# m-schuetz/SimLOD

Measured on NVIDIA H100. Metric: Mpoints/sec octree insertion (16B XYZRGBA), higher is better.
Workload: dtype u32+f32

## Files before the change

### simlod_b200/csrc/construct.cu

```cuda
#include <cooperative_groups.h>
#include <stdint.h>
#include "../../include/simlod_abi.h"
#include "fpmath.cuh"

namespace cg = cooperative_groups;

typedef SimlodPoint Point;
typedef SimlodChunk Chunk;
typedef SimlodNode Node;
typedef SimlodStats Stats;
typedef SimlodUniforms Uniforms;
typedef SimlodHeapHeader Heap;
struct CudaPrint;

#include "construct_layout.cuh"

enum : uint32_t {
    ERR_SPILL_OVERFLOW  = 1u << 0,
    ERR_VOXEL_OVERFLOW  = 1u << 1,
    ERR_DIR_OVERFLOW    = 1u << 2,
    ERR_NODE_OVERFLOW   = 1u << 3,
    ERR_QUEUE_OVERFLOW  = 1u << 4,
    ERR_SPILLNODE_OVERFLOW = 1u << 5,
    ERR_ROW_OVERFLOW    = 1u << 6,
// ... 254 lines not shown
}

constexpr uint32_t PROVISIONAL = 0x80000000u;
static_assert(scratch::ITEM_CAP < (1u << 24), "block-local ranks must fit 24 bits");
constexpr uint32_t CHILD_RANK_BITS = 11;
constexpr uint32_t CHILD_SLOTS = 64 * 8;
__shared__ uint32_t sh_childCount[CHILD_SLOTS];
__shared__ uint8_t  sh_childSplit[CHILD_SLOTS];
__shared__ uint32_t sh_roundSplits;
__device__ __forceinline__ uint32_t childWord(uint32_t e, uint32_t rank) { return PROVISIONAL | (e << CHILD_RANK_BITS) | rank; }
__device__ __forceinline__ uint32_t childOf(uint32_t sl) { return (sl >> CHILD_RANK_BITS) & (CHILD_SLOTS - 1u); }
__device__ __forceinline__ uint32_t finalChildSlot(uint32_t sl) { return (sl & PROVISIONAL) ? sh_childCount[childOf(sl)] + (sl & ((1u << CHILD_RANK_BITS) - 1u)) : sl; }
__shared__ uint32_t sh_leafKey[VOXTAB_SIZE];
__shared__ uint32_t sh_leafCount[VOXTAB_SIZE];
__shared__ uint32_t sh_leafBase[VOXTAB_SIZE];
__shared__ uint8_t  sh_leafLevel[VOXTAB_SIZE];
__device__ __forceinline__ uint32_t finalSlot(uint32_t sl) { return (sl & PROVISIONAL) ? sh_leafBase[(sl >> 24) & 127u] + (sl & 0xffffffu) : sl; }
constexpr uint32_t RUNSLOT_CAP = 2048;
__shared__ uint32_t sh_runSlot[RUNSLOT_CAP];
constexpr uint32_t LIST_CAP = 2048;
static_assert(LIST_CAP <= (1u << CHILD_RANK_BITS), "a child's block-local ranks must fit its slot word");
__shared__ uint32_t sh_listCount;
__shared__ uint32_t sh_listMode;
__shared__ uint32_t sh_blockLegacy;
__shared__ uint8_t  sh_entrySplit[VOXTAB_SIZE];
constexpr uint32_t WL_SPLIT_SHIFT = 22;
constexpr uint32_t WL_ITEM_MASK = (1u << WL_SPLIT_SHIFT) - 1u;
static_assert(scratch::ITEM_CAP <= (1u << WL_SPLIT_SHIFT), "worklist entries keep the item in 22 bits");
__shared__ uint32_t sh_splitNodes[64];
__shared__ SpillInfo sh_splitInfo[64];
__shared__ uint32_t sh_splitGranule[65];
__shared__ uint32_t sh_wlCount, sh_wlBase, sh_wlFill;
__shared__ uint32_t sh_roundLegacy, sh_roundListed;
__device__ __forceinline__ uint32_t blockExclusiveScan(uint32_t v, uint32_t& total) {
    __shared__ uint32_t sh_warpSum[8];
    __shared__ uint32_t sh_total;
    const uint32_t lane = laneId(), warp = threadIdx.x >> 5;
    uint32_t incl = v;
#pragma unroll
    for (int o = 1; o < 32; o <<= 1) { uint32_t t = __shfl_up_sync(0xffffffffu, incl, o); if (lane >= (uint32_t)o) incl += t; }
    __syncthreads();
    if (lane == 31) sh_warpSum[warp] = incl;
    __syncthreads();
    if (threadIdx.x == 0) { uint32_t run = 0; for (int w = 0; w < 8; w++) { uint32_t t = sh_warpSum[w]; sh_warpSum[w] = run; run += t; } sh_total = run; }
    __syncthreads();
    total = sh_total;
    return sh_warpSum[warp] + incl - v;
}

constexpr uint32_t BLOOM_WORDS = 8;
constexpr uint32_t AFFECTED_CAP = 1024;
__shared__ uint32_t sh_runBloom[BLOOM_WORDS];
__shared__ uint32_t sh_affected[AFFECTED_CAP];
__shared__ uint32_t sh_numAffected;
__device__ __forceinline__ uint32_t bloomHash(uint32_t node) { return (node * 0x9E3779B1u) >> 24; }
__device__ __forceinline__ void bloomAdd(uint32_t* bloom, uint32_t node) { uint32_t h = bloomHash(node); atomicOr(&bloom[h >> 5], 1u << (h & 31u)); }

struct Rewalk { uint32_t perRun, runItems, total, spilledBefore; bool listed; };
__device__ __forceinline__ Rewalk rewalkSlice(uint32_t numBatch, uint32_t numSpilled, uint32_t spilledBefore) {
    Rewalk r;
    r.perRun = ((numBatch + gridDim.x - 1) / gridDim.x + 31u) & ~31u;
    r.listed = gridDim.x <= AFFECTED_CAP;
    r.runItems = (r.listed ? sh_numAffected : gridDim.x) * r.perRun;
    r.total = r.runItems + numSpilled;
    r.spilledBefore = spilledBefore;
    return r;
// ... 237 lines not shown
        asm volatile("{\n\t.reg .pred p;\n\tmbarrier.try_wait.parity.shared::cta.b64 p, [%1], %2;\n\tselp.u32 %0, 1, 0, p;\n\t}"
                     : "=r"(done) : "r"(bar), "r"(parity) : "memory");
    } while (!done);
}

__device__ __forceinline__ void blockRun(uint32_t numBatch, uint32_t& first, uint32_t& end) {
    const uint32_t perBlock = ((numBatch + gridDim.x - 1) / gridDim.x + 31u) & ~31u;
    first = min(numBatch, blockIdx.x * perBlock);
    end = min(numBatch, first + perBlock);
}

__device__ __forceinline__ void markAffectedRun(const Ctx& c, const Batch& b, uint32_t spillBegin, uint32_t spillEnd) {
    if (threadIdx.x >= 32) return;
    const uint32_t perRun = ((b.size + gridDim.x - 1) / gridDim.x + 31u) & ~31u;
    uint32_t flag = 0;
    if (blockIdx.x * perRun < b.size) {
        const uint32_t* bloom = c.runBloom() + blockIdx.x * BLOOM_WORDS;
        for (uint32_t k = spillBegin + threadIdx.x; k < spillEnd; k += 32) {
            const uint32_t h = bloomHash(c.spill()[k].node);
            flag |= (ldcg(&bloom[h >> 5]) >> (h & 31u)) & 1u;
        }
        flag = __any_sync(0xffffffffu, flag != 0) ? 1u : 0u;
    }
    if (threadIdx.x == 0) c.runFlag()[blockIdx.x] = flag;
}

__device__ __forceinline__ uint32_t* listItem() { return reinterpret_cast<uint32_t*>(&sh_tile[0][0]); }
__device__ __forceinline__ uint32_t* listSlot() { return reinterpret_cast<uint32_t*>(&sh_tile[0][0]) + LIST_CAP; }
static_assert(sizeof(sh_tile) >= LIST_CAP * 8, "the explicit item list must fit the TMA stages");

__device__ void buildWorklist(const Ctx& c, const Batch& b, uint32_t spillBegin, uint32_t spillEnd, uint32_t round) {
    Ctl::Worklist* w = &c.ctl()->wl[b.index % 3u];
    const uint32_t numSplit = spillEnd - spillBegin;
#ifdef SIMLOD_NO_WORKLIST
    if (true) {
#else
    if (numSplit > 64u || sh_blockLegacy != 0) {
#endif
        if (threadIdx.x == 0) atomicExch(&w->legacy, 1u);
        return;
    }
    uint32_t blockFirst, blockEnd;
    blockRun(b.size, blockFirst, blockEnd);
    const uint32_t mode = sh_listMode;
    const uint32_t total = mode == 0 ? blockEnd - blockFirst : min(sh_listCount, LIST_CAP);
    if (threadIdx.x == 0) { sh_wlCount = 0; sh_wlFill = 0; }
    if (mode == 0) {
        if (threadIdx.x < numSplit) sh_splitNodes[threadIdx.x] = c.spill()[spillBegin + threadIdx.x].node;
        __syncthreads();
        if (threadIdx.x < VOXTAB_SIZE) {
            const uint32_t key = sh_leafKey[threadIdx.x];
            uint32_t f = 0;
            if (key != VOXTAB_EMPTY) for (uint32_t j = 0; j < numSplit; j++) f = key == sh_splitNodes[j] ? j + 1u : f;
            sh_entrySplit[threadIdx.x] = (uint8_t)f;
        }
    } else {
        for (uint32_t e = threadIdx.x; e < CHILD_SLOTS; e += blockDim.x) sh_childSplit[e] = 0;
        __syncthreads();
        if (threadIdx.x < numSplit) {
            const uint32_t node = c.spill()[spillBegin + threadIdx.x].node;
            for (uint32_t k = 0; k < sh_roundSplits; k++) {
                const uint32_t o = node - sh_splitInfo[k].childBase;
                if (o < 8u) sh_childSplit[k * 8u + o] = (uint8_t)(threadIdx.x + 1u);
            }
        }
    }
    __syncthreads();
    const uint32_t* words = mode == 0 ? sh_runSlot : listSlot();
    auto splitOf = [&](uint32_t word) -> uint32_t {
        if ((word & PROVISIONAL) == 0) return 0u;
        return mode == 0 ? sh_entrySplit[(word >> 24) & (VOXTAB_SIZE - 1)] : sh_childSplit[childOf(word)];
    };
    auto movedAt = [&](uint32_t k) { return splitOf(words[k]) != 0; };
    auto wlSplit = [&](uint32_t word) { return (splitOf(word) - 1u) << WL_SPLIT_SHIFT; };
    uint32_t cnt = 0;
    for (uint32_t k = threadIdx.x; k < total; k += blockDim.x) cnt += movedAt(k) ? 1u : 0u;
    for (int o = 16; o > 0; o >>= 1) cnt += __shfl_xor_sync(0xffffffffu, cnt, o);
    if (laneId() == 0 && cnt) atomicAdd(&sh_wlCount, cnt);
    __syncthreads();
    if (threadIdx.x == 0) {
        const uint32_t n = sh_wlCount;
        uint32_t base = n ? atomicAdd(&w->cursor[round & 1u], n) : 0u;
        if ((uint64_t)base + n > scratch::WL_CAP) { atomicExch(&w->legacy, 1u); base = 0xffffffffu; }
        sh_wlBase = base;
    }
    __syncthreads();
    const uint32_t base = sh_wlBase;
    if (base == 0xffffffffu || sh_wlCount == 0) return;
    uint32_t* wl = c.worklist();
    const uint32_t* items = listItem();
    for (uint32_t k0 = 0; k0 < total; k0 += blockDim.x) {
        const uint32_t k = k0 + threadIdx.x;
        const bool m = k < total && movedAt(k);
        const uint32_t mask = __ballot_sync(0xffffffffu, m);
        if (mask == 0) continue;
        uint32_t off = 0;
        if (laneId() == 0) off = atomicAdd(&sh_wlFill, (uint32_t)__popc(mask));
        off = __shfl_sync(0xffffffffu, off, 0);
        if (m) wl[base + off + __popc(mask & lanemaskLt())] = (mode == 0 ? blockFirst + k : items[k]) | wlSplit(words[k]);
    }
}

template <bool SAMPLE, bool COUNT, bool FRESH, bool UNCACHED_GRID>
__device__ __forceinline__ void passItems(const Ctx& c, const Batch& b, uint32_t numSpilled, uint32_t spilledBefore, uint32_t round, uint32_t spillBegin = 0, uint32_t spillEnd = 0) {
    uint32_t blockFirst, blockEnd;
    blockRun(b.size, blockFirst, blockEnd);
    LeafCache cache;
    cache.leaf = VOXTAB_EMPTY; cache.parent = VOXTAB_EMPTY; cache.key = 0;

    if (COUNT && threadIdx.x < VOXTAB_SIZE) { sh_leafKey[threadIdx.x] = VOXTAB_EMPTY; sh_leafCount[threadIdx.x] = 0; }
    if (FRESH && COUNT && threadIdx.x < BLOOM_WORDS) sh_runBloom[threadIdx.x] = 0;
    if (FRESH && COUNT && threadIdx.x == 0) { sh_listMode = 0; sh_listCount = 0; sh_blockLegacy = (blockEnd - blockFirst) > RUNSLOT_CAP ? 1u : 0u; }
    if (SAMPLE) voxelPassBegin(c, b, FRESH);
    __syncthreads();

    if (FRESH) {
        const uint32_t runLen = blockEnd - blockFirst;
        const uint32_t numTiles = (runLen + TILE_POINTS - 1) / TILE_POINTS;
        __syncthreads();
        if (threadIdx.x == 0) asm volatile("fence.proxy.async.shared::cta;" ::: "memory");
        if (threadIdx.x == 0 && numTiles > 0) tileLoad(0, b.points + blockFirst, min(TILE_POINTS, runLen));
        for (uint32_t t = 0; t < numTiles; t++) {
            const uint32_t tileFirst = blockFirst + t * TILE_POINTS;
            if (threadIdx.x == 0 && t + 1 < numTiles)
                tileLoad((t + 1) & 1, b.points + tileFirst + TILE_POINTS, min(TILE_POINTS, blockEnd - (tileFirst + TILE_POINTS)));
            tileWait(t & 1, sh_tilePhase[t & 1] ^ ((t >> 1) & 1u));
#pragma unroll 1
            for (uint32_t k = 0; k < TILE_POINTS / 256; k++) {
                const uint32_t idx = k * 256 + threadIdx.x;
                const uint32_t i = tileFirst + idx;
                const bool valid = i < blockEnd;
                uint4 pt = valid ? sh_tile[t & 1][idx] : make_uint4(0, 0, 0, 0);
                uint32_t lp = 0, slot = 0;
                walk<SAMPLE, COUNT, UNCACHED_GRID, true>(c, b, cache, valid, pt, 0, 0, 0, COUNT ? sh_runBloom : nullptr, false, lp, slot);
                if (valid && COUNT) {
                    c.leafOf(b.parity)[i] = lp;
                    if (runLen <= RUNSLOT_CAP) sh_runSlot[i - blockFirst] = slot; else c.slotOf(b.parity)[i] = slot;
                }
            }
            __syncthreads();
        }
        if (threadIdx.x == 0) { sh_tilePhase[0] ^= ((numTiles + 1) >> 1) & 1u; sh_tilePhase[1] ^= (numTiles >> 1) & 1u; }
        if (COUNT && threadIdx.x < BLOOM_WORDS) c.runBloom()[blockIdx.x * BLOOM_WORDS + threadIdx.x] = sh_runBloom[threadIdx.x];
    } else {
        uint32_t* leafOf = c.leafOf(b.parity);
        uint32_t* slotOf = c.slotOf(b.parity);
        if (sh_roundLegacy == 0) {
            const uint32_t listed = min(sh_roundListed, (uint32_t)scratch::WL_CAP);
            const uint32_t perRun = ((b.size + gridDim.x - 1) / gridDim.x + 31u) & ~31u;
            const uint32_t numSplit = spillEnd - spillBegin;
            if (threadIdx.x < numSplit) sh_splitInfo[threadIdx.x] = c.spill()[spillBegin + threadIdx.x];
            for (uint32_t e = threadIdx.x; e < CHILD_SLOTS; e += blockDim.x) sh_childCount[e] = 0;
            if (threadIdx.x == 0) { sh_listCount = 0; sh_listMode = 1; sh_roundSplits = numSplit; }
            __syncthreads();
            if (threadIdx.x == 0) {
                uint32_t run = 0;
                for (uint32_t k = 0; k < numSplit; k++) { sh_splitGranule[k] = run; run += (sh_splitInfo[k].stored + 31u) / 32u; }
                sh_splitGranule[numSplit] = run;
            }
            __syncthreads();
#if SIMLOD_TIMERS >= 2
            uint64_t tRw = globaltimer();
#define RW_DONE(k) do { __syncthreads(); if (blockIdx.x == 0 && threadIdx.x == 0) { uint64_t _t = globaltimer(); c.ctl()->subNanos[k] += _t - tRw; tRw = _t; } } while (0)
#else
#define RW_DONE(k) do { } while (0)
#endif
            auto reserve = [&](bool valid, bool& forceGlobal) {
                const uint32_t vmask = __ballot_sync(0xffffffffu, valid);
                uint32_t k0 = 0;
                if (laneId() == 0) k0 = atomicAdd(&sh_listCount, (uint32_t)__popc(vmask));
                k0 = __shfl_sync(0xffffffffu, k0, 0);
                forceGlobal = k0 + __popc(vmask) > LIST_CAP;
                if (forceGlobal && laneId() == 0) atomicAdd(&c.ctl()->events[1], 1u);
                return k0 + __popc(vmask & lanemaskLt());
            };
            auto remember = [&](uint32_t i, uint32_t lp, uint32_t slot, uint32_t myk, bool forceGlobal) {
                leafOf[i] = lp;
                if (!forceGlobal) { listItem()[myk] = i; listSlot()[myk] = slot; }
                else {
                    slotOf[i] = slot;
                    if (myk < LIST_CAP) { listItem()[myk] = 0xffffffffu; listSlot()[myk] = 0; }
                }
            };
            RW_DONE(12);
            constexpr uint32_t NO_ITEM = 0xffffffffu;
            auto sampleSplitLeaf = [&](uint64_t grid, const Coords& q, uint32_t color, uint32_t node, uint32_t level) {
                if (!nested(q)) atomicOr(&c.ctl()->errorFlags, ERR_FAR_POINT);
                const uint32_t cell = cellAt(q, level);
                uint32_t* word = reinterpret_cast<uint32_t*>(grid) + (cell >> 5);
                const uint32_t bit = 1u << (cell & 31u);
                const uint32_t seen = (UNCACHED_GRID || SIMLOD_REWALK_L2TEST) ? ldcg(word) : *word;
                if ((seen & bit) == 0 && (atomicOr(word, bit) & bit) == 0) recordVoxel(c, b, node, cell, color);
            };
            {
                const uint32_t share = ((listed + gridDim.x - 1) / gridDim.x + 31u) & ~31u;
                const uint32_t first = min(listed, blockIdx.x * share);
                const uint32_t numListed = min(listed - first, share);
                const uint32_t* wl = c.worklist() + first;
                const uint32_t stride = blockDim.x;
                auto loadEntry = [&](uint32_t bs) { const uint32_t u = bs + laneId(); return u < numListed ? wl[u] : NO_ITEM; };
                auto loadPoint = [&](uint32_t e) {
                    const uint32_t i = e & WL_ITEM_MASK;
                    if (e == NO_ITEM) return make_uint4(0, 0, 0, 0);
                    return i >= scratch::MAX_BATCH ? *reinterpret_cast<const uint4*>(c.spilled() + (i - scratch::MAX_BATCH)) : ldPoint(b.points + i);
                };
                uint32_t base = threadIdx.x & ~31u;
                uint32_t eCur = loadEntry(base), eNext = loadEntry(base + stride);
                uint4 ptCur = loadPoint(eCur);
                for (; base < numListed; base += stride) {
                    const uint4 ptNext = loadPoint(eNext);
                    const uint32_t eNext2 = loadEntry(base + 2u * stride);
                    const uint32_t i = eCur & WL_ITEM_MASK, k = eCur >> WL_SPLIT_SHIFT;
                    const uint4 pt = ptCur;
                    bool valid = eCur != NO_ITEM;
                    const bool spilledItem = valid && i >= scratch::MAX_BATCH;
                    uint32_t node = 0, level = 0, childBase = 0;
                    uint64_t grid = 0;
                    if (valid) {
                        if (k < numSplit) { node = sh_splitInfo[k].node; level = sh_splitInfo[k].level; childBase = sh_splitInfo[k].childBase; grid = sh_splitInfo[k].grid; }
                        else { valid = false; atomicOr(&c.ctl()->errorFlags, ERR_INTERNAL); }
                        valid = valid && level < SIMLOD_MAX_DEPTH;
                    }
                    if (__any_sync(0xffffffffu, valid)) {
                        bool forceGlobal;
                        const uint32_t myk = reserve(valid, forceGlobal);
                        const Coords q = quantize(c, pt);
                        const uint32_t octant = childIndexAt(q, level);
                        const uint32_t child = childBase + octant;
                        if (SAMPLE && valid) sampleSplitLeaf(grid, q, pt.w, node, level);
                        __syncwarp();
                        uint32_t slot = 0;
                        if (COUNT) {
                            uint32_t* bloom = valid && !spilledItem ? c.runBloom() + (i / perRun) * BLOOM_WORDS : nullptr;
                            slot = countChild<false, true>(valid, k * 8u + octant, child, level + 1, bloom, forceGlobal);
                        }
                        if (valid && COUNT) remember(i, child | ((level + 1) << 24), slot, myk, forceGlobal);
                    }
                    eCur = eNext; ptCur = ptNext; eNext = eNext2;
                }
            }
            RW_DONE(13);
            {
                const uint32_t allGranules = sh_splitGranule[numSplit];
                const uint32_t share = (allGranules + gridDim.x - 1) / gridDim.x;
                const uint32_t gFirst = min(allGranules, blockIdx.x * share);
                const uint32_t numGranules = min(allGranules - gFirst, share);
                const uint32_t gStride = blockDim.x / 32u;
                struct Granule { uint32_t lo, j; bool valid; };
                auto locate = [&](uint32_t g) {
                    Granule r; r.lo = 0; r.j = 0; r.valid = false;
                    if (g < numGranules) {
                        const uint32_t ga = gFirst + g;
                        uint32_t lo = 0, hi = numSplit;
                        while (hi - lo > 1) { const uint32_t mid = (lo + hi) >> 1; if (sh_splitGranule[mid] <= ga) lo = mid; else hi = mid; }
                        const uint32_t within = (ga - sh_splitGranule[lo]) * 32u + laneId();
                        r.lo = lo; r.j = sh_splitInfo[lo].base + within;
                        r.valid = within < sh_splitInfo[lo].stored && sh_splitInfo[lo].level < SIMLOD_MAX_DEPTH;
                    }
                    return r;
                };
                auto loadSpilled = [&](const Granule& gr) { return gr.valid ? *reinterpret_cast<const uint4*>(c.spilled() + gr.j) : make_uint4(0, 0, 0, 0); };
                uint32_t g = threadIdx.x >> 5;
                Granule cur = locate(g);
                uint4 ptCur = loadSpilled(cur);
                for (; g < numGranules; g += gStride) {
                    const Granule next = locate(g + gStride);
                    const uint4 ptNext = loadSpilled(next);
                    const bool valid = cur.valid;
                    if (__any_sync(0xffffffffu, valid)) {
                        const uint32_t node = sh_splitInfo[cur.lo].node, level = sh_splitInfo[cur.lo].level, childBase = sh_splitInfo[cur.lo].childBase;
                        const uint32_t i = (uint32_t)scratch::MAX_BATCH + cur.j;
                        const uint4 pt = ptCur;
                        bool forceGlobal;
                        const uint32_t myk = reserve(valid, forceGlobal);
                        const Coords q = quantize(c, pt);
                        const uint32_t octant = childIndexAt(q, level);
                        const uint32_t child = childBase + octant;
                        if (SAMPLE && valid) sampleSplitLeaf(sh_splitInfo[cur.lo].grid, q, pt.w, node, level);
                        __syncwarp();
                        uint32_t slot = 0;
                        if (COUNT) slot = countChild<true, false>(valid, cur.lo * 8u + octant, child, level + 1, nullptr, forceGlobal);
                        if (valid && COUNT) remember(i, child | ((level + 1) << 24), slot, myk, forceGlobal);
                    }
                    cur = next; ptCur = ptNext;
                }
            }
            RW_DONE(14);
        } else {
            if (threadIdx.x == 0) sh_blockLegacy = 1;
            if (first_in_grid()) atomicAdd(&c.ctl()->events[0], 1u);
            if (gridDim.x <= AFFECTED_CAP) {
                const uint32_t* flags = c.runFlag();
                uint32_t numAffected = 0;
                for (uint32_t g0 = 0; g0 < gridDim.x; g0 += blockDim.x) {
                    const uint32_t g = g0 + threadIdx.x;
                    const uint32_t flag = g < gridDim.x ? ldcg(&flags[g]) : 0u;
                    uint32_t total = 0;
                    const uint32_t off = blockExclusiveScan(flag, total);
                    if (flag) sh_affected[numAffected + off] = g;
                    numAffected += total;
                }
                if (threadIdx.x == 0) sh_numAffected = numAffected;
                __syncthreads();
            }
            const Rewalk rw = rewalkSlice(b.size, numSpilled, spilledBefore);
            for (uint32_t base = rewalkFirstGranule(); base < rw.total; base += rewalkGranuleStride()) {
                const uint32_t u = base + laneId();
                uint32_t run = 0xffffffffu, i = 0xffffffffu, node = 0, level = 0;
                bool valid = u < rw.total;
                const bool spilledItem = valid && u >= rw.runItems;
                if (valid) { i = rewalkItem(rw, u, run); valid = spilledItem || i < b.size; }
                uint4 pt = make_uint4(0, 0, 0, 0);
                if (spilledItem) pt = *reinterpret_cast<const uint4*>(c.spilled() + (i - scratch::MAX_BATCH));
                if (valid) {
                    uint32_t lp = leafOf[i];
                    node = lp & 0xffffffu; level = lp >> 24;
                    if (!(spilledItem && i - scratch::MAX_BATCH >= rw.spilledBefore)) valid = c.firstChild()[node] != 0 && level < SIMLOD_MAX_DEPTH;
                }
                if (!__any_sync(0xffffffffu, valid)) continue;
                if (valid && !spilledItem) pt = ldPoint(b.points + i);
// ... 60 lines not shown
                if (sl & PROVISIONAL) slotOf[i] = finalSlot(sl);
            }
        }
    }
    __syncthreads();
}

constexpr uint32_t SPLIT_COPY_PARTS = 256, SPLIT_CLEAR_PARTS = 32, SPLIT_PARTS = SPLIT_COPY_PARTS + SPLIT_CLEAR_PARTS + 1;

__device__ __noinline__ void splitRound(uint32_t begin, uint32_t end) {
    const Ctx c;
    const Batch& b = sh_batch;
    const uint32_t numWarps = (gridDim.x * blockDim.x) >> 5;
    const uint32_t warp = (threadIdx.x >> 5) * gridDim.x + blockIdx.x;
    const uint32_t lane = laneId();
    const uint32_t numItems = (end - begin) * SPLIT_PARTS;
    uint32_t* leafOf = c.leafOf(b.parity);
    for (uint32_t item = warp; item < numItems; item += numWarps) {
        const SpillInfo info = c.spill()[begin + item / SPLIT_PARTS];
        const uint32_t part = item % SPLIT_PARTS;
        const uint32_t numChunks = (info.stored + SIMLOD_POINTS_PER_CHUNK - 1) / SIMLOD_POINTS_PER_CHUNK;
        if (part < SPLIT_COPY_PARTS) {
            const uint32_t k = part >> 2, quarter = part & 3u;
            if (k >= numChunks || info.row == 0) continue;
            const Chunk* chunk = reinterpret_cast<const Chunk*>(c.rows()[(uint64_t)(info.row - 1) * scratch::ROW_SLOTS + k]);
            const uint32_t inChunk = min((uint32_t)SIMLOD_POINTS_PER_CHUNK, info.stored - k * SIMLOD_POINTS_PER_CHUNK);
            const uint32_t first = quarter * 256u;
            const uint32_t n = inChunk > first ? min(256u, inChunk - first) : 0u;
            const uint32_t tag = info.node | (info.level << 24);
            const uint4* src = reinterpret_cast<const uint4*>(&chunk->points[first]);
            const uint32_t dst = info.base + k * SIMLOD_POINTS_PER_CHUNK + first;
#pragma unroll 1
            for (uint32_t h = 0; h < 256u; h += 128u) {
                uint4 v[4];
#pragma unroll
                for (int u = 0; u < 4; u++) if (h + lane + 32u * u < n) v[u] = src[h + lane + 32u * u];
#pragma unroll
                for (int u = 0; u < 4; u++) if (h + lane + 32u * u < n) {
                    *reinterpret_cast<uint4*>(c.spilled() + dst + h + lane + 32u * u) = v[u];
                    leafOf[scratch::MAX_BATCH + dst + h + lane + 32u * u] = tag;
                }
            }
        } else if (part < SPLIT_COPY_PARTS + SPLIT_CLEAR_PARTS) {
            constexpr uint32_t PER = SIMLOD_GRID_WORDS / 4 / SPLIT_CLEAR_PARTS;
            uint4* g = reinterpret_cast<uint4*>(info.grid) + (uint64_t)(part - SPLIT_COPY_PARTS) * PER;
#pragma unroll 4
            for (uint32_t i = lane; i < PER; i += 32) g[i] = make_uint4(0, 0, 0, 0);
        } else {
            Node* parent = &c.nodes()[info.node];
            const uint32_t pX = parent->X, pY = parent->Y, pZ = parent->Z;
            if (lane < 8) {
                Node* child = &c.nodes()[info.childBase + lane];
                uint64_t* raw = reinterpret_cast<uint64_t*>(child);
#pragma unroll
                for (int w = 0; w < 19; w++) raw[w] = 0;
                child->level = info.level + 1;
                child->X = 2 * pX + ((lane >> 2) & 1);
                child->Y = 2 * pY + ((lane >> 1) & 1);
                child->Z = 2 * pZ + (lane & 1);
                for (int k = 0; k < 20; k++) child->name[k] = parent->name[k];
                reinterpret_cast<uint8_t*>(child)[offsetof(Node, name) + info.level + 1] = (uint8_t)('0' + lane);
                child->isLeaf = 1;
                parent->children[lane] = child;
                c.firstChild()[info.childBase + lane] = 0;
                c.parentOf()[info.childBase + lane] = info.node;
                c.gridPtr()[info.childBase + lane] = 0;
                c.leafRow()[info.childBase + lane] = 0;
// ... 329 lines not shown
        float sy = fpx::sub(uniforms.boxMax[1], uniforms.boxMin[1]);
        float sz = fpx::sub(uniforms.boxMax[2], uniforms.boxMin[2]);
        l.size = fmaxf(fmaxf(sx, sy), sz);
        l.rcpSize = fpx::rcp(l.size);
        l.minx = uniforms.boxMin[0]; l.miny = uniforms.boxMin[1]; l.minz = uniforms.boxMin[2];
        sh_launch = l;
        sh_loop.tStart = globaltimer();
        sh_allocTarget = 0; sh_allocSeen = 0; sh_numAffected = 0;
    }

    if (first_in_grid()) {
        *frameStartTimestamp = sh_loop.tStart;
        ctl->numBatchesUploaded = *(volatile uint32_t*)numBatchesUploaded_volatile;
        ctl->elapsedNanos = 0; ctl->elapsedByParity[0] = 0; ctl->elapsedByParity[1] = 0;
        ctl->memUsed = c.heap()->offset;
        ctl->freshBytes = 0;
        ctl->allocDone = 0;
        for (int i = 0; i < 3; i++) { clearBatchCounters(&ctl->batch[i]); clearWorklist(&ctl->wl[i]); }
        for (int i = 0; i < 8; i++) ctl->statCounters[i] = 0;
        if (stats->batchletIndex == 0) {
            ctl->errorFlags = 0;
            ctl->spilledTotal = 0; ctl->voxelsTotal = 0; ctl->voxelsByPass[0] = 0; ctl->voxelsByPass[1] = 0;
            for (int i = 0; i < 8; i++) ctl->phaseNanos[i] = 0;
            for (int i = 0; i < 16; i++) ctl->subNanos[i] = 0;
            ctl->launchCount = 0;
            for (int i = 0; i < 4; i++) ctl->events[i] = 0;
            for (int i = 0; i < 12; i++) for (int j = 0; j < 4; j++) ctl->roundHist[i][j] = 0;
            ctl->rowBump = 0; ctl->rowFreeCount = 0;
            c.firstChild()[0] = 0;
            c.parentOf()[0] = 0;
            c.leafRow()[0] = 0;
            c.splitState()[0] = 0;
            c.gridPtr()[0] = (uint64_t)nodes[0].grid;
        }
    }
    tileBarInit();
    gridSync();
#if SIMLOD_TIMERS >= 1
    uint64_t tPhase = sh_loop.tStart;
#define PHASE_DONE(k) do { if (first_in_grid()) { uint64_t _t = globaltimer(); ctl->phaseNanos[k] += _t - tPhase; tPhase = _t; tSub = _t; } } while (0)
    uint64_t tSub = tPhase;
#else
#define PHASE_DONE(k) do { } while (0)
#endif
#if SIMLOD_TIMERS >= 2
#define SUB_DONE(k) do { if (first_in_grid()) { uint64_t _t = globaltimer(); ctl->subNanos[k] += _t - tSub; tSub = _t; } } while (0)
#else
#define SUB_DONE(k) do { } while (0)
#endif
    PHASE_DONE(7);

    if (threadIdx.x == 0) {
        const uint32_t numBatchesUploaded = ldv(&ctl->numBatchesUploaded);
        const uint32_t firstBatch = ldv(&stats->batchletIndex);
        sh_loop.firstBatch = firstBatch;
        sh_loop.lastBatch = firstBatch + min(numBatchesUploaded - firstBatch, 20u);
        sh_loop.havePending = 0;
        sh_loop.pendingAllocated = 0;
        sh_loop.allocEpochs = 0;
    }
    __syncthreads();
    auto nextSize = [&](uint32_t batchIndex) { return batchIndex + 1 < sh_loop.lastBatch ? &batchSizes[(batchIndex + 1) % SIMLOD_BATCH_STREAM_SIZE] : nullptr; };

    if (sh_loop.lastBatch > sh_loop.firstBatch) takeSnapshot(c, &ctl->batch[sh_loop.firstBatch % 3u], sh_loop.firstBatch & 1u, &batchSizes[sh_loop.firstBatch % SIMLOD_BATCH_STREAM_SIZE]);
    for (uint32_t batchIndex = sh_loop.firstBatch; batchIndex < sh_loop.lastBatch; batchIndex++) {
        if (threadIdx.x == 0) {
            Batch b;
            b.size = min(sh_snap.nextBatchSize, (uint32_t)SIMLOD_MAX_BATCH_SIZE);
            b.points = sh_launch.ring + (uint64_t)(batchIndex % SIMLOD_BATCH_STREAM_SIZE) * SIMLOD_MAX_BATCH_SIZE;
            b.index = batchIndex;
            b.parity = batchIndex & 1u;
            b.bc = &ctl->batch[batchIndex % 3u];
            sh_batch = b;
            sh_loop.deferSampling = sh_snap.rootFirstChild == 0 ? 1u : 0u;
        }
        __syncthreads();
        const Batch& b = sh_batch;

        uint64_t memUsed = sh_snap.memUsed;
        if (sh_loop.havePending && memUsed + (uint64_t)sh_snap.numSpillTotal * SIMLOD_GRID_STRIDE + sh_loop.pendingBound + HEAP_GUARD_BYTES >= uniforms.persistentBufferCapacity) {
            allocateChunks();
            gridSync();
// ... 4 lines not shown
        }
        const bool memCapacityReached = memUsed + HEAP_GUARD_BYTES >= uniforms.persistentBufferCapacity;
        if (first_in_grid()) stats->memCapacityReached = memCapacityReached ? 1 : 0;
        if (memCapacityReached) break;

        const float elapsedMs = float(sh_snap.elapsedNanos) / 1000000.0f;
        if (batchIndex > sh_loop.firstBatch && elapsedMs > 10.0f) break;

        SUB_DONE(11);
        if (sh_loop.havePending && !sh_loop.pendingAllocated) {
            if (threadIdx.x == 0) { const uint32_t epoch = ++sh_loop.allocEpochs; sh_allocTarget = epoch * gridDim.x; sh_allocSeen = 0; }
            __syncthreads();
            allocateChunks();
            __syncthreads();
            if (threadIdx.x == 0) { __threadfence(); atomicAdd(&ctl->allocDone, 1u); }
        }
        SUB_DONE(0);
        if (first_in_grid()) { clearBatchCounters(&ctl->batch[(batchIndex + 1) % 3u]); clearWorklist(&ctl->wl[(batchIndex + 1) % 3u]); }
        if (sh_loop.deferSampling) passItems<false, true, true, false>(c, b, 0, 0, 0);
        else               passItems<true, true, true, false>(c, b, 0, 0, 0);
        SUB_DONE(1);
        waitAllocBlock(c);
        SUB_DONE(2);
        if (sh_loop.deferSampling) passFlush<false, true, true>(c, b, 0, 0);
        else               passFlush<true, true, true>(c, b, 0, 0);
        SUB_DONE(3);
        if (sh_loop.havePending) {
            if (first_in_grid()) finishBatchBookkeeping(c, sh_loop.pending, sh_loop.pendingBound);
            insertAll();
            if (threadIdx.x == 0) { sh_allocTarget = 0; sh_loop.havePending = 0; }
        }
        if (first_in_grid()) { const uint64_t el = globaltimer() - sh_loop.tStart; ctl->elapsedNanos = el; ctl->elapsedByParity[b.parity] = el; }
        SUB_DONE(4);
        gridSync();
        takeSnapshot(c, b.bc, b.parity, nextSize(batchIndex));
        SUB_DONE(5);
        PHASE_DONE(0);

        uint32_t spillBegin = 0, spilledBefore = 0;
        for (int round = 0; round < 24; round++) {
            const uint32_t spillEnd = min(sh_snap.numSpillTotal, (uint32_t)scratch::SPILLNODE_CAP);
            if (spillEnd == spillBegin) break;
#if SIMLOD_TIMERS >= 2
            const uint64_t tRound = first_in_grid() ? globaltimer() : 0ull;
#endif
            markAffectedRun(c, b, spillBegin, spillEnd);
            buildWorklist(c, b, spillBegin, spillEnd, (uint32_t)round);
            splitRound(spillBegin, spillEnd);
            SUB_DONE(6);
            gridSync();
            SUB_DONE(7);
            PHASE_DONE(1);
#if SIMLOD_TIMERS >= 1
            if (first_in_grid()) ctl->phaseNanos[6] += 1;
#endif
            const uint32_t numSpilled = min(sh_snap.numSpilled, (uint32_t)scratch::SPILL_CAP);
            if (threadIdx.x == 0) {
                Ctl::Worklist* w = &ctl->wl[batchIndex % 3u];
                const uint32_t lg = ldv(&w->legacy), nl = ldv(&w->cursor[round & 1]);
                sh_roundLegacy = lg; sh_roundListed = nl;
            }
            if (first_in_grid()) ctl->wl[batchIndex % 3u].cursor[(round + 1) & 1] = 0;
            __syncthreads();
            if (sh_loop.deferSampling) passItems<false, true, false, false>(c, b, numSpilled, spilledBefore, (uint32_t)round, spillBegin, spillEnd);
            else               passItems<true, true, false, false>(c, b, numSpilled, spilledBefore, (uint32_t)round, spillBegin, spillEnd);
            SUB_DONE(8);
            if (sh_loop.deferSampling) passFlush<false, true, false>(c, b, numSpilled, spilledBefore);
            else               passFlush<true, true, false>(c, b, numSpilled, spilledBefore);
            SUB_DONE(9);
            gridSync();
#if SIMLOD_TIMERS >= 2
            if (first_in_grid()) {
                const uint32_t listed = sh_roundLegacy ? 0u : min(sh_roundListed, (uint32_t)scratch::WL_CAP), moved = numSpilled - spilledBefore;
                const uint32_t cls = min(11u, (32u - (uint32_t)__clz(listed + moved)) / 2u);
                ctl->roundHist[cls][0] += 1; ctl->roundHist[cls][1] += globaltimer() - tRound; ctl->roundHist[cls][2] += listed; ctl->roundHist[cls][3] += moved;
            }
#endif
            takeSnapshot(c, b.bc, b.parity, nextSize(batchIndex));
            SUB_DONE(10);
            PHASE_DONE(2);
            spillBegin = spillEnd;
            spilledBefore = numSpilled;
        }
        const uint32_t numSpilled = min(sh_snap.numSpilled, (uint32_t)scratch::SPILL_CAP);
        if (sh_loop.deferSampling) {
            passItems<true, false, true, true>(c, b, numSpilled, 0, 0);
            passFlush<true, false, true>(c, b, numSpilled, 0);
            gridSync();
            takeSnapshot(c, b.bc, b.parity, nextSize(batchIndex));
            PHASE_DONE(3);
        }
        if (threadIdx.x == 0) {
            sh_loop.havePending = 1;
            sh_loop.pending = b;
            sh_loop.pendingSpilled = numSpilled;
            sh_loop.pendingBacklog = min(sh_snap.numBacklog, (uint32_t)scratch::VOXEL_SHARED);
            sh_loop.pendingBound = chunkAllocationBound(b.size);
            sh_loop.pendingAllocated = 0;
        }
    }
    __syncthreads();

    if (sh_loop.havePending) {
// ... 51 lines not shown
```

### simlod_b200/csrc/construct_layout.cuh

```cuda
#pragma once
#include <stddef.h>
#include <stdint.h>
#include "../../include/simlod_abi.h"

constexpr uint64_t HEAP_GUARD_BYTES = 200000000ull;

namespace scratch {
constexpr uint64_t NODE_CAP       = 263157;
constexpr uint64_t NODE_TAB       = 263168;
constexpr uint64_t MAX_BATCH      = SIMLOD_MAX_BATCH_SIZE;
constexpr uint64_t SPILL_CAP      = 3ull << 20;
constexpr uint64_t ITEM_CAP       = MAX_BATCH + SPILL_CAP;
constexpr uint64_t VOXEL_CAP      = 4ull << 20;
constexpr uint64_t VOXEL_SHARED   = 512ull << 10;
constexpr uint64_t DIR_CAP        = 512ull << 10;
constexpr uint64_t QUEUE_CAP      = 3ull << 19;
constexpr uint64_t WL_CAP         = 2ull << 20;
constexpr uint64_t SPILLNODE_CAP  = 100000;
constexpr uint64_t ROW_CAP        = 65536;
constexpr uint64_t ROW_SLOTS      = 64;
constexpr uint64_t BLOCK_CAP      = 4096;

constexpr uint64_t align256(uint64_t x) { return (x + 255) & ~255ull; }
constexpr uint64_t OFF_CTL        = 0;
// ... 23 lines not shown
constexpr uint64_t TOTAL          = align256(OFF_WORKLIST + WL_CAP * 4);
static_assert(TOTAL <= 300000000ull, "scratch must fit the host's 300 MB momentary buffer (main.cpp:554)");
}

struct BatchCounters {
    uint32_t numSpillTotal;
    uint32_t numSpilled;
    uint32_t numBacklog;
    uint32_t numDirtyLeaves;
    uint32_t numDirtyVox;
    uint32_t dirCursor;
    uint32_t voxelsCreated;
    uint32_t insertCursor;
};

struct Ctl {
    uint32_t numBatchesUploaded;
    uint32_t errorFlags;
    uint64_t elapsedNanos;
    uint64_t memUsed;
    uint32_t rowBump;
    uint32_t rowFreeCount;
    uint32_t statCounters[8];
    uint64_t voxelsByPass[2];
    uint64_t spilledTotal;
    uint64_t voxelsTotal;
    uint64_t phaseNanos[8];
    BatchCounters batch[3];
    uint32_t allocDone;
    uint32_t _pad[3];
    uint64_t launchClock[32][2];
    uint32_t launchCount, _pad2[3];
    uint64_t subNanos[16];
    struct Worklist { uint32_t cursor[2]; uint32_t legacy; uint32_t pad; } wl[3];
    uint32_t events[4];
    uint64_t elapsedByParity[2];
    uint64_t roundHist[12][4];
    uint64_t heapExact;
    uint64_t freshBytes;
};
static_assert(offsetof(Ctl, roundHist) == 1008 && offsetof(Ctl, freshBytes) == 1400 && sizeof(Ctl) <= 4096, "tools read Ctl by offset; the control block is 4 KB");
static_assert(offsetof(Ctl, events) == 976, "tools read Ctl by offset");
static_assert(offsetof(Ctl, spilledTotal) == 80, "bench.py reads Ctl::spilledTotal at byte 80");
static_assert(offsetof(Ctl, phaseNanos) == 96 && offsetof(Ctl, batch) == 160 && offsetof(Ctl, allocDone) == 256 && offsetof(Ctl, launchClock) == 272 && offsetof(Ctl, launchCount) == 784 && offsetof(Ctl, subNanos) == 800, "tools read Ctl by offset");

struct SpillInfo {
    uint32_t node;
    uint32_t stored;
    uint32_t base;
    uint32_t row;
    uint32_t childBase;
    uint32_t level;
    uint64_t grid;
};
static_assert(sizeof(SpillInfo) == 32, "SpillInfo");

struct DirEntry { uint32_t base; uint32_t k0; };
```

Baseline: 6387.

## Add guided dynamic chunking of split-round work across blocks

Each block now takes only a fixed share (three quarters) of the listed worklist entries and spilled granules in the split round. The remainder is handed out in small chunks through a global atomic tail counter, so blocks that finish early pick up more work. The aim is to reduce load imbalance and the wait at the grid barrier that follows. It also adds optional barrier-spread timing instrumentation behind SIMLOD_TIMERS, and costs extra block syncs and atomics per chunk.

```diff
diff --git a/simlod_b200/csrc/construct.cu b/simlod_b200/csrc/construct.cu
--- a/simlod_b200/csrc/construct.cu
+++ b/simlod_b200/csrc/construct.cu
@@ -310,6 +310,17 @@
 __shared__ uint32_t sh_splitGranule[65];
 __shared__ uint32_t sh_wlCount, sh_wlBase, sh_wlFill;
 __shared__ uint32_t sh_roundLegacy, sh_roundListed;
+constexpr uint32_t FIXED_QUARTERS = 3;
+constexpr uint32_t CHUNK_UNITS = 8;
+struct GuidedShares {
+    uint32_t fixedListed, fixedGranules;
+    uint32_t listedTail, granuleTail;
+    uint32_t listedUnits, units;
+};
+__shared__ GuidedShares sh_guided;
+__shared__ uint32_t sh_tailUnit;
+struct Segment { uint32_t first, numListed, gFirst, numGranules; };
+__shared__ Segment sh_segment;
 __device__ __forceinline__ uint32_t blockExclusiveScan(uint32_t v, uint32_t& total) {
     __shared__ uint32_t sh_warpSum[8];
     __shared__ uint32_t sh_total;
@@ -613,6 +624,7 @@
 __device__ void buildWorklist(const Ctx& c, const Batch& b, uint32_t spillBegin, uint32_t spillEnd, uint32_t round) {
     Ctl::Worklist* w = &c.ctl()->wl[b.index % 3u];
     const uint32_t numSplit = spillEnd - spillBegin;
+    if (first_in_grid()) w->tail = 0;
 #ifdef SIMLOD_NO_WORKLIST
     if (true) {
 #else
@@ -679,6 +691,26 @@
         if (laneId() == 0) off = atomicAdd(&sh_wlFill, (uint32_t)__popc(mask));
         off = __shfl_sync(0xffffffffu, off, 0);
         if (m) wl[base + off + __popc(mask & lanemaskLt())] = (mode == 0 ? blockFirst + k : items[k]) | wlSplit(words[k]);
+    }
+}
+
+__device__ __noinline__ void takeChunk() {
+    const Ctx c;
+    const Batch& b = sh_batch;
+    const GuidedShares& gs = sh_guided;
+    const uint32_t n = min(CHUNK_UNITS, (LIST_CAP - min(sh_listCount, LIST_CAP)) / 32u);
+    const uint32_t k = n ? atomicAdd(&c.ctl()->wl[b.index % 3u].tail, n) : 0xffffffffu;
+    sh_tailUnit = k;
+    sh_segment.numListed = 0; sh_segment.numGranules = 0;
+    if (k < gs.listedUnits) {
+        const uint32_t listed = min(sh_roundListed, (uint32_t)scratch::WL_CAP);
+        sh_segment.first = gs.listedTail + k * 32u;
+        sh_segment.numListed = min(listed, gs.listedTail + min(k + n, gs.listedUnits) * 32u) - sh_segment.first;
+    }
+    if (k < gs.units && k + n > gs.listedUnits) {
+        const uint32_t g0 = max(k, gs.listedUnits);
+        sh_segment.gFirst = gs.granuleTail + (g0 - gs.listedUnits);
+        sh_segment.numGranules = min(k + n, gs.units) - g0;
     }
 }
 
@@ -727,17 +759,31 @@
         uint32_t* leafOf = c.leafOf(b.parity);
         uint32_t* slotOf = c.slotOf(b.parity);
         if (sh_roundLegacy == 0) {
-            const uint32_t listed = min(sh_roundListed, (uint32_t)scratch::WL_CAP);
+            const uint32_t numSplit = spillEnd - spillBegin;
             const uint32_t perRun = ((b.size + gridDim.x - 1) / gridDim.x + 31u) & ~31u;
-            const uint32_t numSplit = spillEnd - spillBegin;
             if (threadIdx.x < numSplit) sh_splitInfo[threadIdx.x] = c.spill()[spillBegin + threadIdx.x];
             for (uint32_t e = threadIdx.x; e < CHILD_SLOTS; e += blockDim.x) sh_childCount[e] = 0;
             if (threadIdx.x == 0) { sh_listCount = 0; sh_listMode = 1; sh_roundSplits = numSplit; }
             __syncthreads();
             if (threadIdx.x == 0) {
+                const uint32_t listed = min(sh_roundListed, (uint32_t)scratch::WL_CAP);
                 uint32_t run = 0;
                 for (uint32_t k = 0; k < numSplit; k++) { sh_splitGranule[k] = run; run += (sh_splitInfo[k].stored + 31u) / 32u; }
                 sh_splitGranule[numSplit] = run;
+                const uint32_t shareL = ((listed + gridDim.x - 1) / gridDim.x + 31u) & ~31u, shareG = (run + gridDim.x - 1) / gridDim.x;
+                const bool guided = (uint64_t)listed + 32ull * run <= (uint64_t)gridDim.x * (LIST_CAP - 32u);
+                GuidedShares gs;
+                gs.fixedListed = guided ? (shareL * FIXED_QUARTERS / 4u) & ~31u : shareL;
+                gs.fixedGranules = guided ? shareG * FIXED_QUARTERS / 4u : shareG;
+                gs.listedTail = min(listed, gridDim.x * gs.fixedListed);
+                gs.granuleTail = min(run, gridDim.x * gs.fixedGranules);
+                gs.listedUnits = (listed - gs.listedTail + 31u) / 32u;
+                gs.units = gs.listedUnits + (run - gs.granuleTail);
+                sh_guided = gs;
+                sh_segment.first = min(listed, blockIdx.x * gs.fixedListed);
+                sh_segment.numListed = min(listed - sh_segment.first, gs.fixedListed);
+                sh_segment.gFirst = min(run, blockIdx.x * gs.fixedGranules);
+                sh_segment.numGranules = min(run - sh_segment.gFirst, gs.fixedGranules);
             }
             __syncthreads();
 #if SIMLOD_TIMERS >= 2
@@ -773,100 +819,102 @@
                 const uint32_t seen = (UNCACHED_GRID || SIMLOD_REWALK_L2TEST) ? ldcg(word) : *word;
                 if ((seen & bit) == 0 && (atomicOr(word, bit) & bit) == 0) recordVoxel(c, b, node, cell, color);
             };
-            {
-                const uint32_t share = ((listed + gridDim.x - 1) / gridDim.x + 31u) & ~31u;
-                const uint32_t first = min(listed, blockIdx.x * share);
-                const uint32_t numListed = min(listed - first, share);
-                const uint32_t* wl = c.worklist() + first;
-                const uint32_t stride = blockDim.x;
-                auto loadEntry = [&](uint32_t bs) { const uint32_t u = bs + laneId(); return u < numListed ? wl[u] : NO_ITEM; };
-                auto loadPoint = [&](uint32_t e) {
-                    const uint32_t i = e & WL_ITEM_MASK;
-                    if (e == NO_ITEM) return make_uint4(0, 0, 0, 0);
-                    return i >= scratch::MAX_BATCH ? *reinterpret_cast<const uint4*>(c.spilled() + (i - scratch::MAX_BATCH)) : ldPoint(b.points + i);
-                };
-                uint32_t base = threadIdx.x & ~31u;
-                uint32_t eCur = loadEntry(base), eNext = loadEntry(base + stride);
-                uint4 ptCur = loadPoint(eCur);
-                for (; base < numListed; base += stride) {
-                    const uint4 ptNext = loadPoint(eNext);
-                    const uint32_t eNext2 = loadEntry(base + 2u * stride);
-                    const uint32_t i = eCur & WL_ITEM_MASK, k = eCur >> WL_SPLIT_SHIFT;
-                    const uint4 pt = ptCur;
-                    bool valid = eCur != NO_ITEM;
-                    const bool spilledItem = valid && i >= scratch::MAX_BATCH;
-                    uint32_t node = 0, level = 0, childBase = 0;
-                    uint64_t grid = 0;
-                    if (valid) {
-                        if (k < numSplit) { node = sh_splitInfo[k].node; level = sh_splitInfo[k].level; childBase = sh_splitInfo[k].childBase; grid = sh_splitInfo[k].grid; }
-                        else { valid = false; atomicOr(&c.ctl()->errorFlags, ERR_INTERNAL); }
-                        valid = valid && level < SIMLOD_MAX_DEPTH;
+            for (;;) {
+                {
+                    const uint32_t first = sh_segment.first, numListed = sh_segment.numListed;
+                    const uint32_t* wl = c.worklist() + first;
+                    const uint32_t stride = blockDim.x;
+                    auto loadEntry = [&](uint32_t bs) { const uint32_t u = bs + laneId(); return u < numListed ? wl[u] : NO_ITEM; };
+                    auto loadPoint = [&](uint32_t e) {
+                        const uint32_t i = e & WL_ITEM_MASK;
+                        if (e == NO_ITEM) return make_uint4(0, 0, 0, 0);
+                        return i >= scratch::MAX_BATCH ? *reinterpret_cast<const uint4*>(c.spilled() + (i - scratch::MAX_BATCH)) : ldPoint(b.points + i);
+                    };
+                    uint32_t base = threadIdx.x & ~31u;
+                    uint32_t eCur = loadEntry(base), eNext = loadEntry(base + stride);
+                    uint4 ptCur = loadPoint(eCur);
+                    for (; base < numListed; base += stride) {
+                        const uint4 ptNext = loadPoint(eNext);
+                        const uint32_t eNext2 = loadEntry(base + 2u * stride);
+                        const uint32_t i = eCur & WL_ITEM_MASK, k = eCur >> WL_SPLIT_SHIFT;
+                        const uint4 pt = ptCur;
+                        bool valid = eCur != NO_ITEM;
+                        const bool spilledItem = valid && i >= scratch::MAX_BATCH;
+                        uint32_t node = 0, level = 0, childBase = 0;
+                        uint64_t grid = 0;
+                        if (valid) {
+                            if (k < numSplit) { node = sh_splitInfo[k].node; level = sh_splitInfo[k].level; childBase = sh_splitInfo[k].childBase; grid = sh_splitInfo[k].grid; }
+                            else { valid = false; atomicOr(&c.ctl()->errorFlags, ERR_INTERNAL); }
+                            valid = valid && level < SIMLOD_MAX_DEPTH;
+                        }
+                        if (__any_sync(0xffffffffu, valid)) {
+                            bool forceGlobal;
+                            const uint32_t myk = reserve(valid, forceGlobal);
+                            const Coords q = quantize(c, pt);
+                            const uint32_t octant = childIndexAt(q, level);
+                            const uint32_t child = childBase + octant;
+                            if (SAMPLE && valid) sampleSplitLeaf(grid, q, pt.w, node, level);
+                            __syncwarp();
+                            uint32_t slot = 0;
+                            if (COUNT) {
+                                uint32_t* bloom = valid && !spilledItem ? c.runBloom() + (i / perRun) * BLOOM_WORDS : nullptr;
+                                slot = countChild<false, true>(valid, k * 8u + octant, child, level + 1, bloom, forceGlobal);
+                            }
+                            if (valid && COUNT) remember(i, child | ((level + 1) << 24), slot, myk, forceGlobal);
+                        }
+                        eCur = eNext; ptCur = ptNext; eNext = eNext2;
                     }
-                    if (__any_sync(0xffffffffu, valid)) {
-                        bool forceGlobal;
-                        const uint32_t myk = reserve(valid, forceGlobal);
-                        const Coords q = quantize(c, pt);
-                        const uint32_t octant = childIndexAt(q, level);
-                        const uint32_t child = childBase + octant;
-                        if (SAMPLE && valid) sampleSplitLeaf(grid, q, pt.w, node, level);
-                        __syncwarp();
-                        uint32_t slot = 0;
-                        if (COUNT) {
-                            uint32_t* bloom = valid && !spilledItem ? c.runBloom() + (i / perRun) * BLOOM_WORDS : nullptr;
-                            slot = countChild<false, true>(valid, k * 8u + octant, child, level + 1, bloom, forceGlobal);
+                }
+                RW_DONE(13);
+                {
+                    const uint32_t gFirst = sh_segment.gFirst, numGranules = sh_segment.numGranules;
+                    const uint32_t gStride = blockDim.x / 32u;
+                    struct Granule { uint32_t lo, j; bool valid; };
+                    auto locate = [&](uint32_t g) {
+                        Granule r; r.lo = 0; r.j = 0; r.valid = false;
+                        if (g < numGranules) {
+                            const uint32_t ga = gFirst + g;
+                            uint32_t lo = 0, hi = numSplit;
+                            while (hi - lo > 1) { const uint32_t mid = (lo + hi) >> 1; if (sh_splitGranule[mid] <= ga) lo = mid; else hi = mid; }
+                            const uint32_t within = (ga - sh_splitGranule[lo]) * 32u + laneId();
+                            r.lo = lo; r.j = sh_splitInfo[lo].base + within;
+                            r.valid = within < sh_splitInfo[lo].stored && sh_splitInfo[lo].level < SIMLOD_MAX_DEPTH;
                         }
-                        if (valid && COUNT) remember(i, child | ((level + 1) << 24), slot, myk, forceGlobal);
+                        return r;
+                    };
+                    auto loadSpilled = [&](const Granule& gr) { return gr.valid ? *reinterpret_cast<const uint4*>(c.spilled() + gr.j) : make_uint4(0, 0, 0, 0); };
+                    uint32_t g = threadIdx.x >> 5;
+                    Granule cur = locate(g);
+                    uint4 ptCur = loadSpilled(cur);
+                    for (; g < numGranules; g += gStride) {
+                        const Granule next = locate(g + gStride);
+                        const uint4 ptNext = loadSpilled(next);
+                        const bool valid = cur.valid;
+                        if (__any_sync(0xffffffffu, valid)) {
+                            const uint32_t node = sh_splitInfo[cur.lo].node, level = sh_splitInfo[cur.lo].level, childBase = sh_splitInfo[cur.lo].childBase;
+                            const uint32_t i = (uint32_t)scratch::MAX_BATCH + cur.j;
+                            const uint4 pt = ptCur;
+                            bool forceGlobal;
+                            const uint32_t myk = reserve(valid, forceGlobal);
+                            const Coords q = quantize(c, pt);
+                            const uint32_t octant = childIndexAt(q, level);
+                            const uint32_t child = childBase + octant;
+                            if (SAMPLE && valid) sampleSplitLeaf(sh_splitInfo[cur.lo].grid, q, pt.w, node, level);
+                            __syncwarp();
+                            uint32_t slot = 0;
+                            if (COUNT) slot = countChild<true, false>(valid, cur.lo * 8u + octant, child, level + 1, nullptr, forceGlobal);
+                            if (valid && COUNT) remember(i, child | ((level + 1) << 24), slot, myk, forceGlobal);
+                        }
+                        cur = next; ptCur = ptNext;
                     }
-                    eCur = eNext; ptCur = ptNext; eNext = eNext2;
                 }
-            }
-            RW_DONE(13);
-            {
-                const uint32_t allGranules = sh_splitGranule[numSplit];
-                const uint32_t share = (allGranules + gridDim.x - 1) / gridDim.x;
-                const uint32_t gFirst = min(allGranules, blockIdx.x * share);
-                const uint32_t numGranules = min(allGranules - gFirst, share);
-                const uint32_t gStride = blockDim.x / 32u;
-                struct Granule { uint32_t lo, j; bool valid; };
-                auto locate = [&](uint32_t g) {
-                    Granule r; r.lo = 0; r.j = 0; r.valid = false;
-                    if (g < numGranules) {
-                        const uint32_t ga = gFirst + g;
-                        uint32_t lo = 0, hi = numSplit;
-                        while (hi - lo > 1) { const uint32_t mid = (lo + hi) >> 1; if (sh_splitGranule[mid] <= ga) lo = mid; else hi = mid; }
-                        const uint32_t within = (ga - sh_splitGranule[lo]) * 32u + laneId();
-                        r.lo = lo; r.j = sh_splitInfo[lo].base + within;
-                        r.valid = within < sh_splitInfo[lo].stored && sh_splitInfo[lo].level < SIMLOD_MAX_DEPTH;
-                    }
-                    return r;
-                };
-                auto loadSpilled = [&](const Granule& gr) { return gr.valid ? *reinterpret_cast<const uint4*>(c.spilled() + gr.j) : make_uint4(0, 0, 0, 0); };
-                uint32_t g = threadIdx.x >> 5;
-                Granule cur = locate(g);
-                uint4 ptCur = loadSpilled(cur);
-                for (; g < numGranules; g += gStride) {
-                    const Granule next = locate(g + gStride);
-                    const uint4 ptNext = loadSpilled(next);
-                    const bool valid = cur.valid;
-                    if (__any_sync(0xffffffffu, valid)) {
-                        const uint32_t node = sh_splitInfo[cur.lo].node, level = sh_splitInfo[cur.lo].level, childBase = sh_splitInfo[cur.lo].childBase;
-                        const uint32_t i = (uint32_t)scratch::MAX_BATCH + cur.j;
-                        const uint4 pt = ptCur;
-                        bool forceGlobal;
-                        const uint32_t myk = reserve(valid, forceGlobal);
-                        const Coords q = quantize(c, pt);
-                        const uint32_t octant = childIndexAt(q, level);
-                        const uint32_t child = childBase + octant;
-                        if (SAMPLE && valid) sampleSplitLeaf(sh_splitInfo[cur.lo].grid, q, pt.w, node, level);
-                        __syncwarp();
-                        uint32_t slot = 0;
-                        if (COUNT) slot = countChild<true, false>(valid, cur.lo * 8u + octant, child, level + 1, nullptr, forceGlobal);
-                        if (valid && COUNT) remember(i, child | ((level + 1) << 24), slot, myk, forceGlobal);
-                    }
-                    cur = next; ptCur = ptNext;
-                }
-            }
-            RW_DONE(14);
+                RW_DONE(14);
+                if (sh_guided.units == 0) break;
+                __syncthreads();
+                if (threadIdx.x == 0) takeChunk();
+                __syncthreads();
+                if (sh_tailUnit >= sh_guided.units) break;
+            }
         } else {
             if (threadIdx.x == 0) sh_blockLegacy = 1;
             if (first_in_grid()) atomicAdd(&c.ctl()->events[0], 1u);
@@ -993,7 +1041,7 @@
             const uint32_t dst = info.base + k * SIMLOD_POINTS_PER_CHUNK + first;
 #pragma unroll 1
             for (uint32_t h = 0; h < 256u; h += 128u) {
-                uint4 v[4];
+                uint4 v[4] = {};
 #pragma unroll
                 for (int u = 0; u < 4; u++) if (h + lane + 32u * u < n) v[u] = src[h + lane + 32u * u];
 #pragma unroll
@@ -1389,7 +1437,14 @@
             c.leafRow()[0] = 0;
             c.splitState()[0] = 0;
             c.gridPtr()[0] = (uint64_t)nodes[0].grid;
-        }
+#if SIMLOD_TIMERS >= 1
+            for (int i = 0; i < 3; i++) for (int j = 0; j < 3; j++) ctl->spreadNanos[i][j] = 0;
+#endif
+        }
+#if SIMLOD_TIMERS >= 1
+        ctl->spreadBase = sh_loop.tStart;
+        for (int i = 0; i < 2; i++) { ctl->barrierSlot[i].first = ~0ull; ctl->barrierSlot[i].last = 0; ctl->barrierSlot[i].sum = 0; ctl->barrierSlot[i].count = 0; }
+#endif
     }
     tileBarInit();
     gridSync();
@@ -1405,6 +1460,32 @@
 #else
 #define SUB_DONE(k) do { } while (0)
 #endif
+#if SIMLOD_TIMERS >= 1
+    uint32_t timedBarriers = 0;
+    auto timedGridSync = [&](uint32_t type) {
+        Ctl::BarrierSlot* s = &ctl->barrierSlot[timedBarriers & 1u];
+        __syncthreads();
+        if (threadIdx.x == 0) {
+            const uint64_t t = globaltimer() - ldv(&ctl->spreadBase);
+            atomicMin(reinterpret_cast<unsigned long long*>(&s->first), (unsigned long long)t);
+            atomicMax(reinterpret_cast<unsigned long long*>(&s->last), (unsigned long long)t);
+            atomicAdd(reinterpret_cast<unsigned long long*>(&s->sum), (unsigned long long)t);
+            atomicAdd(&s->count, 1u);
+        }
+        gridSync();
+        if (first_in_grid()) {
+            const uint64_t first = ldv(&s->first), last = ldv(&s->last), sum = ldv(&s->sum);
+            const uint32_t n = ldv(&s->count);
+            ctl->spreadNanos[type][0] += 1;
+            ctl->spreadNanos[type][1] += last - first;
+            ctl->spreadNanos[type][2] += last - sum / n;
+            s->first = ~0ull; s->last = 0; s->sum = 0; s->count = 0;
+        }
+        timedBarriers++;
+    };
+#else
+    auto timedGridSync = [](uint32_t) { gridSync(); };
+#endif
     PHASE_DONE(7);
 
     if (threadIdx.x == 0) {
@@ -1475,7 +1556,7 @@
         }
         if (first_in_grid()) { const uint64_t el = globaltimer() - sh_loop.tStart; ctl->elapsedNanos = el; ctl->elapsedByParity[b.parity] = el; }
         SUB_DONE(4);
-        gridSync();
+        timedGridSync(0);
         takeSnapshot(c, b.bc, b.parity, nextSize(batchIndex));
         SUB_DONE(5);
         PHASE_DONE(0);
@@ -1491,7 +1572,7 @@
             buildWorklist(c, b, spillBegin, spillEnd, (uint32_t)round);
             splitRound(spillBegin, spillEnd);
             SUB_DONE(6);
-            gridSync();
+            timedGridSync(1);
             SUB_DONE(7);
             PHASE_DONE(1);
 #if SIMLOD_TIMERS >= 1
@@ -1511,7 +1592,7 @@
             if (sh_loop.deferSampling) passFlush<false, true, false>(c, b, numSpilled, spilledBefore);
             else               passFlush<true, true, false>(c, b, numSpilled, spilledBefore);
             SUB_DONE(9);
-            gridSync();
+            timedGridSync(2);
 #if SIMLOD_TIMERS >= 2
             if (first_in_grid()) {
                 const uint32_t listed = sh_roundLegacy ? 0u : min(sh_roundListed, (uint32_t)scratch::WL_CAP), moved = numSpilled - spilledBefore;
diff --git a/simlod_b200/csrc/construct_layout.cuh b/simlod_b200/csrc/construct_layout.cuh
--- a/simlod_b200/csrc/construct_layout.cuh
+++ b/simlod_b200/csrc/construct_layout.cuh
@@ -79,14 +79,18 @@
     uint64_t launchClock[32][2];
     uint32_t launchCount, _pad2[3];
     uint64_t subNanos[16];
-    struct Worklist { uint32_t cursor[2]; uint32_t legacy; uint32_t pad; } wl[3];
+    struct Worklist { uint32_t cursor[2]; uint32_t legacy; uint32_t tail; } wl[3];
     uint32_t events[4];
     uint64_t elapsedByParity[2];
     uint64_t roundHist[12][4];
     uint64_t heapExact;
     uint64_t freshBytes;
+    uint64_t spreadBase;
+    struct BarrierSlot { uint64_t first, last, sum; uint32_t count, pad; } barrierSlot[2];
+    uint64_t spreadNanos[3][3];
 };
 static_assert(offsetof(Ctl, roundHist) == 1008 && offsetof(Ctl, freshBytes) == 1400 && sizeof(Ctl) <= 4096, "tools read Ctl by offset; the control block is 4 KB");
+static_assert(offsetof(Ctl, barrierSlot) == 1416 && offsetof(Ctl, spreadNanos) == 1480, "tools read Ctl by offset");
 static_assert(offsetof(Ctl, events) == 976, "tools read Ctl by offset");
 static_assert(offsetof(Ctl, spilledTotal) == 80, "bench.py reads Ctl::spilledTotal at byte 80");
 static_assert(offsetof(Ctl, phaseNanos) == 96 && offsetof(Ctl, batch) == 160 && offsetof(Ctl, allocDone) == 256 && offsetof(Ctl, launchClock) == 272 && offsetof(Ctl, launchCount) == 784 && offsetof(Ctl, subNanos) == 800, "tools read Ctl by offset");
```

After: 6437 (median of 6 runs). No clear change (+0.8%).
